# DrSleep/nas-segm-pytorch

Hardware: AMD Instinct MI355X
Metric: images/sec (fwd+bwd+optimizer step) WACV arch0 2048x1024 bs=4/GPU (higher is better)
Workload: dtype f32

## Files before the change

### include/nasseg.h

```cpp
#ifndef NASSEG_H
#define NASSEG_H

#include <stdint.h>

#ifdef __cplusplus
extern "C" {
#endif

const char* nasseg_last_error(void);
int nasseg_abi_version(void);
int nasseg_device_count(void);

int nasseg_dw_pack_weight(const float* w, float* wt, int C, int K, int flip, void* stream);
int nasseg_dwconv(const float* x, const float* wt, float* y, const float* in_scale,
                  const float* in_shift, int in_act, const float* scale, const float* shift, int act,
                  int B, int H, int W, int C, int Ho, int Wo, int K, int stride, int pad, int dil,
                  int transposed, float* stats, void* stream);
int nasseg_dwconv_strip_ok(int K, int stride, int dil);
int64_t nasseg_dwconv_stats_blocks(int B, int C, int Ho, int Wo, int K, int stride, int dil);
int nasseg_dwconv_bwd_data_bn(const float* dy, const float* wt, float* g, const float* z,
                              const float* scale, const float* shift, const float* mean,
                              const float* invstd, int act, int B, int H, int W, int C, int Ho,
                              int Wo, int K, int stride, int pad, int dil, int transposed,
                              float* stats, void* stream);
// ... 63 lines not shown
                            int dil, float* stats, void* stream);
int nasseg_conv_wgrad_lds3x3(int B, int Hs, int Ws, int K, int Ho, int Wo, int N, int kh, int kw, int stride,
                             int pad, int dil);
int64_t nasseg_conv_wgrad_workspace(int B, int Ho, int Wo, int N, int K, int kh, int kw);
int nasseg_wgrad_finalize_many(int count, const float* const* partial, float* const* dw,
                               const int* dims, void* stream);
int nasseg_conv_wgrad_many(int count, const int64_t* desc, void* stream);
int nasseg_dwconv_wgrad_many(int count, const int64_t* desc, void* stream);

int nasseg_conv_wgrad_bn(const float* x, int ldx, const float* g, int ldg, const float* z, int ldz, float* dz,
                         int lddz, float* dw, float* ws, const float* in_scale, const float* in_shift, int in_act,
                         const float* bn_scale, const float* bn_shift, const float* bn_mean, const float* bn_invstd,
                         const float* bn_sums, int bn_train, int bn_act, int B, int H, int W, int K, int N, void* stream);
int nasseg_conv_wgrad_bn_flat(const float* x, int ldx, const float* g, int ldg, const float* z, int ldz, float* dw,
                              float* ws, const float* bn_scale, const float* bn_shift, const float* bn_mean,
                              const float* bn_invstd, const float* bn_sums, int bn_train, int bn_act, int B, int Hs,
                              int Ws, int K, int Ho, int Wo, int N, int kh, int kw, int stride, int pad, int dil,
                              void* stream);
int nasseg_dwconv_wgrad_bn(const float* x, const float* g, const float* z, float* dz, float* dw, float* ws,
                           const float* in_scale, const float* in_shift, int in_act, const float* bn_scale, const float* bn_shift,
                           const float* bn_mean, const float* bn_invstd, const float* bn_sums, int bn_train, int bn_act,
                           int B, int H, int W, int C, int Ho, int Wo, int K, int stride, int pad, int dil,
                           void* stream);
int64_t nasseg_conv_pw_bwd_slabs(int B, int H, int W, int K, int N);
int64_t nasseg_conv_pw_bwd_reads_z(int B, int H, int W, int K, int N);
int64_t nasseg_conv_pw_bwd_kernel_id(int B, int H, int W, int K, int N, int z_null);
int64_t nasseg_conv_pw_bwd_rz_min_pixels(int64_t v);
int nasseg_conv_pw_bwd_bn(const float* x, const float* g, const float* z, const float* wb, float* dx, float* dw,
                          float* ws, const float* in_scale, const float* in_shift, int in_act, int dx_act,
                          const float* bn_scale, const float* bn_shift, const float* bn_mean, const float* bn_invstd,
                          const float* bn_sums, int bn_train, int bn_act, int B, int H, int W, int K, int N,
                          const float* in_mean, const float* in_invstd, float* dx_stats, const float* dx_res,
                          void* stream);
int nasseg_conv_wgrad(const float* x, int ldx, const float* dy, int lddy, float* dw, float* ws,
                      const float* in_scale, const float* in_shift, int in_act, int B, int Hs,
                      int Ws, int K, int Ho, int Wo, int N, int kh, int kw, int stride, int pad,
                      int dil, void* stream);

int64_t nasseg_colred_workspace(int S, int64_t R, int C);
int nasseg_colred(int mode, const float* a, int64_t lda, const float* b, int64_t ldb,
                  const float* c, int64_t ldc, float* out, float* ws, int S, int64_t R, int C,
                  float mul, void* stream);
int nasseg_bn_stats(const float* x, int64_t ldx, int64_t M, int C, float eps, float momentum,
                    const float* gamma, const float* beta, float* mean, float* invstd,
                    float* scale, float* shift, float* running_mean, float* running_var,
                    int64_t* num_batches_tracked, float* ws, void* stream);
int nasseg_bn_finalize(float* partial, int nblk, int64_t M, int C, float eps, float momentum,
                       const float* gamma, const float* beta, float* mean, float* invstd,
                       float* scale, float* shift, float* running_mean, float* running_var,
                       int64_t* num_batches_tracked, void* stream);
int nasseg_bn_eval_params(int C, float eps, const float* gamma, const float* beta,
                          const float* running_mean, const float* running_var, float* mean,
                          float* invstd, float* scale, float* shift, void* stream);
int nasseg_bn_bwd_reduce(const float* dy, int64_t lddy, const float* x, int64_t ldx, int64_t M,
                         int C, const float* scale, const float* shift, const float* mean,
                         const float* invstd, int act, float* sums, float* ws, void* stream);
int nasseg_rows_sum(float* partial, int nblk, int cols, float* out, void* stream);
int nasseg_bn_bwd_apply(const float* dy, const float* x, const float* scale, const float* shift,
                        const float* mean, const float* invstd, const float* sums, int64_t M,
                        int C, int train, int act, float* dx, void* stream);
int64_t nasseg_colred_rows(int S, int64_t R, int C);
int64_t nasseg_bn_bwd_apply_rows_max_bytes(void);
int nasseg_bn_bwd_reduce_rows(const float* dy, int64_t lddy, const float* x, int64_t ldx, int64_t M, int C,
                              const float* scale, const float* shift, const float* mean, const float* invstd, int act,
                              float* rows, void* stream);
int nasseg_bn_bwd_apply_rows(const float* dy, const float* x, const float* scale, const float* shift, const float* mean,
// ... 258 lines not shown
typedef struct nasseg_bf16_t {
  uint16_t v;
} nasseg_bf16_t;
int nasseg_to_bf16(const float* x, nasseg_bf16_t* y, int64_t n, void* stream);
int nasseg_from_bf16(const nasseg_bf16_t* x, float* y, int64_t n, void* stream);
int nasseg_bf16_irdw_stats(const nasseg_bf16_t* x, const float* w1, const float* in_scale, const float* in_shift,
                           int in_act, int B, int H, int W, int K, int C, float eps, float momentum, const float* gamma,
                           const float* beta, float* mean, float* invstd, float* scale, float* shift,
                           float* running_mean, float* running_var, int64_t* num_batches_tracked, float* ws,
                           void* stream);
int nasseg_bf16_irdw_fwd(const nasseg_bf16_t* x, const float* w1, const float* wdw, nasseg_bf16_t* z2,
                         const float* in_scale, const float* in_shift, int in_act, const float* bn1_scale,
                         const float* bn1_shift, int act1, int B, int H, int W, int K, int C, int Ho, int Wo, int stride,
                         float* stats, void* stream);
int nasseg_bf16_irdw_bwd(const nasseg_bf16_t* x, const float* w1, const nasseg_bf16_t* g, const nasseg_bf16_t* z2,
                         const float* wdw, int wdw_flipped, nasseg_bf16_t* ge, float* dw, float* ws,
                         const float* in_scale, const float* in_shift, int in_act, const float* bn1_scale,
                         const float* bn1_shift, const float* bn1_mean, const float* bn1_invstd, int act1,
                         const float* bn2_scale, const float* bn2_shift, const float* bn2_mean,
                         const float* bn2_invstd, const float* bn2_sums, int bn2_train, int bn2_act, int B, int H, int W,
                         int K, int C, int Ho, int Wo, int stride, float* stats, void* stream);
int nasseg_bf16_dwconv_bwd_bn(const nasseg_bf16_t* xz, const nasseg_bf16_t* g, const nasseg_bf16_t* z, const float* wt,
                              int wt_flipped, nasseg_bf16_t* ge, float* dw, float* ws, const float* in_scale, const float* in_shift,
                              const float* in_mean, const float* in_invstd, int in_act, const float* bn_scale,
                              const float* bn_shift, const float* bn_mean, const float* bn_invstd, const float* bn_sums,
                              int bn_train, int bn_act, int B, int H, int W, int C, int Ho, int Wo, int K, int stride,
                              int pad, int dil, float* stats, void* stream);
int nasseg_bf16_conv_pw_bwd_bn(const nasseg_bf16_t* x, const nasseg_bf16_t* g, const nasseg_bf16_t* z, const float* wb,
                               nasseg_bf16_t* dx, float* dw, float* ws, const float* in_scale, const float* in_shift,
                               int in_act, int dx_act, const float* bn_scale, const float* bn_shift, const float* bn_mean,
                               const float* bn_invstd, const float* bn_sums, int bn_train, int bn_act, int B, int H,
                               int W, int K, int N, const float* in_mean, const float* in_invstd, float* dx_stats,
                               const nasseg_bf16_t* dx_res, void* stream);
int nasseg_bf16_sepconv_fwd(const nasseg_bf16_t* x, const float* wdw, const float* wpw, nasseg_bf16_t* zdw,
                            nasseg_bf16_t* y, const float* in_scale, const float* in_shift, int in_act,
                            const float* out_scale, const float* out_shift, int out_act, int B, int H, int W, int C,
                            int Ho, int Wo, int N, int K, int stride, int pad, int dil, float* stats, void* stream);
int nasseg_bf16_affine_act(const nasseg_bf16_t* x, const float* scale, const float* shift, const nasseg_bf16_t* res,
                      nasseg_bf16_t* y, int64_t n, int C, int act, void* stream);
int nasseg_bf16_psum_bwd(const nasseg_bf16_t* dy, const nasseg_bf16_t* za, const float* tsa, int act_a, const float* ca,
                         nasseg_bf16_t* ga, float* part_a, const nasseg_bf16_t* zb, const float* tsb, int act_b,
                         const float* cb, nasseg_bf16_t* gb, float* part_b, float* cpart, int B, int H, int W, int C,
                         void* stream);
int nasseg_bf16_add_act2(const nasseg_bf16_t* xa, const float* sa, const float* ha, int act_a, const float* ca,
                         const nasseg_bf16_t* xb, const float* sb, const float* hb, int act_b, const float* cb,
                         nasseg_bf16_t* y, int64_t n, int C, void* stream);
int nasseg_bf16_bn_bwd_apply(const nasseg_bf16_t* dy, const nasseg_bf16_t* x, const float* scale, const float* shift,
                        const float* mean, const float* invstd, const float* sums, int64_t M,
                        int C, int train, int act, nasseg_bf16_t* dx, void* stream);
int nasseg_bf16_bn_bwd_reduce_rows(const nasseg_bf16_t* dy, int64_t lddy, const nasseg_bf16_t* x, int64_t ldx, int64_t M,
                                   int C, const float* scale, const float* shift, const float* mean, const float* invstd,
                                   int act, float* rows, void* stream);
int nasseg_bf16_bn_bwd_apply_rows(const nasseg_bf16_t* dy, const nasseg_bf16_t* x, const float* scale, const float* shift,
                                  const float* mean, const float* invstd, const float* rows, int nrows, float* sums_out,
                                  int64_t M, int C, int train, int act, nasseg_bf16_t* dx, void* stream);
int nasseg_bf16_grad_junction(const nasseg_bf16_t* g0, const nasseg_bf16_t* g1, const nasseg_bf16_t* g2,
                              const nasseg_bf16_t* g3, const nasseg_bf16_t* g4, const nasseg_bf16_t* g5,
                              const nasseg_bf16_t* g6, const nasseg_bf16_t* g7, int n, const nasseg_bf16_t* z,
                              const float* tstats, int act, nasseg_bf16_t* out, float* part, int B, int H, int W, int C,
                              void* stream);
int nasseg_bf16_axpby(const nasseg_bf16_t* a, const nasseg_bf16_t* b, const float* alpha, const float* beta, nasseg_bf16_t* y,
                 int64_t n, int C, int act, void* stream);
int nasseg_bf16_act_bwd(const nasseg_bf16_t* dy, const nasseg_bf16_t* ref, nasseg_bf16_t* dx, int64_t n, int act, void* stream);
int nasseg_bf16_fill(nasseg_bf16_t* y, int64_t n, float v, void* stream);
int nasseg_bf16_chan_copy(const nasseg_bf16_t* x, int64_t ldx, int xoff, nasseg_bf16_t* y, int64_t ldy, int yoff,
                     const nasseg_bf16_t* mref, int64_t ldm, int moff, int64_t P, int C, int act, int mact,
// ... 230 lines not shown
```

### nas-segm-pytorch_amd/csrc/conv_pwbwd.hip

```cpp
#include <atomic>
#include <cstdlib>
#include <type_traits>

#include "conv_common.h"

#if NASSEG_FP32_ONLY
std::atomic<int64_t> g_pw_rz_min_pixels{1 << 18};
#else
extern std::atomic<int64_t> g_pw_rz_min_pixels;
#endif

namespace {

#ifndef NASSEG_PW_CHUNK
#define NASSEG_PW_CHUNK 3
#endif
#ifndef NASSEG_PW_RECOMPUTE_Z
#define NASSEG_PW_RECOMPUTE_Z 1
#endif
constexpr int kPwTile = 64;
constexpr int kPwMaxTiles = 24;

struct PwArgs {
  const act_t* x;
  const act_t* g;
  const act_t* z;
  act_t* dx;
  float* partial;
  const float* wb;
  const float* in_scale;
  const float* in_shift;
  int in_act;
  const float* bn_scale;
  const float* bn_shift;
  const float* bn_mean;
  const float* bn_invstd;
  const float* bn_sums;
  int bn_train, bn_act;
  float invM;
  int dx_act;
  const float* in_mean;
  const float* in_invstd;
// ... 510 lines not shown
#pragma unroll
                for (int q = 0; q < NQ; ++q) acc[q] = mfma16(av, bv[q], acc[q]);
              }
            };
            switch (c) {
              case 0: dw_chunk(acc2[0]); break;
              case 1: dw_chunk(acc2[1]); break;
              case 2: if constexpr (KC > 2) dw_chunk(acc2[2]); break;
              case 3: if constexpr (KC > 3) dw_chunk(acc2[3]); break;
              case 4: if constexpr (KC > 4) dw_chunk(acc2[4]); break;
              default: if constexpr (KC > 5) dw_chunk(acc2[5]); break;
            }
          }
        };
        if (nq >= 4) mfma_phase(std::integral_constant<int, 4>());
        else if (nq == 3) mfma_phase(std::integral_constant<int, 3>());
        else if (nq == 2) mfma_phase(std::integral_constant<int, 2>());
        else mfma_phase(std::integral_constant<int, 1>());
      }
    }
  }
  if (own) {
    float* pout = a.partial + (int64_t)blockIdx.x * N * K;
#pragma unroll
    for (int c = 0; c < KC; ++c)
#pragma unroll
      for (int q = 0; q < 4; ++q)
#pragma unroll
        for (int r = 0; r < 4; ++r) {
          const int n = wave * 16 + 4 * kg + r, k = c * kPwChunk + q * 16 + j;
          if (n < N && k < K) pout[(int64_t)n * K + k] = acc2[c][q][r];
        }
  }
}

struct PwPlan {
  int ok, nt, kt, nslab, pix_per_slab, wide, rz;
};
inline int pw_round_nt(int nt) {
  const int allowed[] = {2, 3, 4, 6, 9, 12};
  for (int v : allowed)
    if (nt <= v) return v;
  return 0;
}
inline PwPlan pw_plan(int64_t M, int N, int K) {
  PwPlan p = {};
  if (N % 4 || K % 4 || N <= 0 || K <= 0 || M <= 0 || M >= 2147483647LL) return p;
  const int kt0 = cdiv(K, 16);
  p.kt = kt0 <= 1 ? 1 : (kt0 <= 2 ? 2 : (kt0 <= 4 ? 4 : 0));
  p.nt = pw_round_nt(cdiv(N, 16));
  if (!p.kt || !p.nt || p.nt * p.kt > kPwMaxTiles) {
    if (N > 64 || K > 384) return p;
    p.wide = 1;
    p.nt = cdiv(N, 16);
    p.kt = cdiv(K, kPwChunk);
  }
  const int64_t lds = p.wide ? (int64_t)(32 << 10)
                             : (int64_t)pw_lds_floats(p.nt, p.kt, pw_weight_in_lds(p.nt, p.kt)) * 4;
  int64_t s = lds > (40 << 10) ? 512 : 1024;
  const int64_t cap = (int64_t)((p.wide ? 64 : 16) << 20) / ((int64_t)N * K * 4);
  while (s > 1 && (s > cap || s > M / (4 * kPwTile))) s >>= 1;
  if (!p.wide && s < 256 && M / kPwTile > s) {
    s = M / kPwTile < 256 ? M / kPwTile : 256;
    if (s > cap) s = cap;
    if (s < 1) s = 1;
  }
// ... 128 lines not shown
    switch (id - kPwIdWide) {
      case 2: PW_WIDE(2); break;
      case 3: PW_WIDE(3); break;
      case 4: PW_WIDE(4); break;
      case 5: PW_WIDE(5); break;
      case 6: PW_WIDE(6); break;
      default: return nasseg_fail(NASSEG_ERR_UNSUPPORTED, "conv_pw_bwd_bn: no kernel with id %d", id);
    }
#undef PW_WIDE
    NASSEG_LAUNCH_CHECK("conv_pw_bwd_wide_kernel");
    if (!dw) return NASSEG_OK;
    const float* parts_w[1] = {ws};
    float* outs_w[1] = {dw};
    const int dims_w[5] = {p.nslab, 1, N, K, 0};
    return nasseg_wgrad_finalize_many(1, parts_w, outs_w, dims_w, stream);
  }
  switch (id) {
#define X(NT_, KT_) case pw_id(NT_, KT_, 1): pw_launch<NT_, KT_, true>(a, p.nslab, pro, s); break;
    PW_REBUILD(X)
#undef X
#define X(NT_, KT_) case pw_id(NT_, KT_, 0): pw_launch<NT_, KT_>(a, p.nslab, pro, s); break;
    PW_NARROW(X)
#undef X
    default: return nasseg_fail(NASSEG_ERR_UNSUPPORTED, "conv_pw_bwd_bn: no kernel with id %d", id);
  }
  NASSEG_LAUNCH_CHECK("conv_pw_bwd_kernel");
  if (!dw) return NASSEG_OK;
  const float* parts[1] = {ws};
  float* outs[1] = {dw};
  const int dims[5] = {p.nslab, 1, N, K, 0};
  return nasseg_wgrad_finalize_many(1, parts, outs, dims, stream);
}

}
```

### nas-segm-pytorch_amd/functional.py

```python
import collections
import ctypes
import os
import weakref

import numpy as np
import torch

from ._lib import LaunchProfiler, NassegError, current_stream, lib, ptr, require_device

ACT_NONE, ACT_RELU, ACT_RELU6 = 0, 1, 2
RED_SUM, RED_SUMSQ, RED_DOT2, RED_DOT1 = 0, 1, 3, 4


_BF16_PREFIX = "nasseg_bf16_"


def _k(name, t):
    if t.dtype == torch.float32:
        return name
    return _BF16_PREFIX + name[7:]


def _to_dtype(t, dtype):
    if t.dtype == dtype:
# ... 221 lines not shown

def _dense_wgrad(cur, dz, w, psc, psh, pact, geom):
    B, Hs, Ws, K, Ho, Wo, N, kh, kw, stride, pad, dil = geom
    dwt = torch.empty_like(w)
    ws = _ws(cur, lib.query("nasseg_conv_wgrad_workspace", B, Ho, Wo, N, K, kh, kw))
    flat = int(lib.query("nasseg_conv_fwd_pack_mode", K, kh, kw) == 2)
    if (deferred_wgrad.active and (B * Hs * Ws * K + B * Ho * Wo * N) * cur.element_size() <= _GROUP_WGRAD_BYTES
            and not (psc is None and psh is None and not pact
                     and lib.query("nasseg_conv_wgrad_lds3x3", B, Hs, Ws, K, Ho, Wo, N, kh, kw, stride, pad, dil))):
        desc = (ptr(cur), K, ptr(dz), N, ptr(ws), ptr(psc) or 0, ptr(psh) or 0, pact) + tuple(geom)
        _group_wgrad("nasseg_conv_wgrad_many", cur, (cur, dz, psc, psh, ws), desc,
                     _fin_entry(ws, dwt, kh * kw, N, K, flat))
        return dwt
    st = _wgrad_stream(cur, (cur, dz, psc, psh, ws))
    lib.call(_k("nasseg_conv_wgrad", cur), ptr(cur), K, ptr(dz), N, _finish_wgrad(ws, dwt, kh * kw, N, K, flat),
             ptr(ws), ptr(psc), ptr(psh), pact, *geom, st)
    return dwt


def _pw_bwd_slabs(kind, cur, z, w, stride, pad, need_dw, need_dx, i, ops):
    if not (FUSE_PW_BWD and kind == "dense" and need_dw and need_dx):
        return 0
    N, K, kh, kw = w.shape
    if not (kh == 1 and kw == 1 and stride == 1 and pad == 0):
        return 0
    if (cur.numel() + z.numel()) * cur.element_size() <= _PW_BWD_MIN_BYTES:
        return 0
    if K % 4 == 0 and i > 0 and ops[i - 1].has_bn and not (N >= K and K <= 64):
        return 0
    B, _, H, W = cur.shape
    if K > 64 and not (_PW_BWD_WIDE and B * H * W >= _PW_BWD_WIDE_MIN_PIXELS):
        return 0
    return lib.query("nasseg_conv_pw_bwd_slabs", B, H, W, K, N)


FUSE_DW_BWD = os.environ.get("NASSEG_FUSE_DW_BWD", "1") != "0"
_DW_BWD_MIN_BYTES = int(os.environ.get("NASSEG_DW_BWD_MIN_BYTES", 24 << 20))
_FLAT_WGRAD_BN_MIN_BYTES = 24 << 20


def _dw_bwd_rows(kind, cur, z, w, stride, pad, dil, need_dw, need_dx, i, ops):
    if not (FUSE_DW_BWD and kind == "dw" and need_dw and need_dx and i > 0 and ops[i - 1].has_bn):
        return 0
    if (cur.numel() + z.numel()) * cur.element_size() <= _DW_BWD_MIN_BYTES:
        return 0
    B, C, H, W = cur.shape
    return lib.query("nasseg_dwconv_bwd_bn_rows", B, C, H, W, w.shape[-1], stride, pad, dil)


def _flat_bn_ok(kind, need_dw, need_dx, psc, psh, pact, w, N, z):
    return (kind == "dense" and need_dw and not need_dx and psc is None and psh is None and not pact
            and w.shape[2] * w.shape[3] > 1 and N % 4 == 0
            and lib.query("nasseg_conv_fwd_pack_mode", w.shape[1], w.shape[2], w.shape[3]) == 2
            and z.numel() * z.element_size() > _FLAT_WGRAD_BN_MIN_BYTES)


def _wgrad_bn_ok(kind, cur, z, w, stride, pad, dil):
    if (cur.numel() + z.numel()) * cur.element_size() <= _GROUP_WGRAD_BYTES:
        return False
    K, N = cur.shape[1], z.shape[1]
    if kind == "dw":
        return K % 4 == 0 and bool(lib.query("nasseg_dwconv_strip_ok", w.shape[-1], stride, dil))
    return (w.shape[2] == 1 and w.shape[3] == 1 and stride == 1 and pad == 0 and K % 4 == 0 and N % 4 == 0)


def _wgrad_bn(kind, cur, g, z, w, psc, psh, pact, bn, geom):
# ... 336 lines not shown
        geom = (B, Ho, Wo, C, H, W, K, stride, pad, dil, 1)
    if bn is not None:
        nb = lib.query("nasseg_dwconv_bwd_data_bn_blocks", B, C, H, W, K, geom[7], geom[8], dil, geom[10])
        if nb > 0:
            z, scale, shift, mean, invstd, act = bn
            part = _rows_ws(dz, nb, C)
            lib.call(_k("nasseg_dwconv_bwd_data_bn", dz), ptr(dz), ptr(wt), ptr(dx), ptr(z), ptr(scale),
                     ptr(shift), ptr(mean), ptr(invstd), act, *geom, ptr(part), s)
            return dx, (part, nb)
    lib.call(_k("nasseg_dwconv", dz), ptr(dz), ptr(wt), ptr(dx), None, None, ACT_NONE, None, None,
             ACT_NONE, *geom, None, s)
    return dx, None


_IDENTITY = {}


def _identity_vectors(like, n):
    key = (like.device, (n + 1023) // 1024)
    ent = _IDENTITY.get(key)
    if ent is None:
        m = key[1] * 1024
        ent = (torch.ones(m, device=like.device, dtype=torch.float32),
               torch.zeros(m, device=like.device, dtype=torch.float32))
        _IDENTITY[key] = ent
    return ent


FUSE_RES_GRAD = os.environ.get("NASSEG_FUSE_RES_GRAD", "1") != "0"
FUSE_PW_BWD = os.environ.get("NASSEG_FUSE_PW_BWD", "1") != "0"
_PW_BWD_MIN_BYTES = int(os.environ.get("NASSEG_PW_BWD_MIN_BYTES", 24 << 20))
_PW_BWD_WIDE = os.environ.get("NASSEG_PW_BWD_WIDE", "1") == "1"
_PW_BWD_WIDE_MIN_PIXELS = 1 << 16
FUSE_BN_RELU_CONV = os.environ.get("NASSEG_FUSE_BN_RELU_CONV", "1") != "0"
FUSE_POOL_BN = os.environ.get("NASSEG_FUSE_POOL_BN", "1") != "0"
FUSE_CAT_REDUCE = os.environ.get("NASSEG_FUSE_CAT_REDUCE", "1") != "0"
FUSE_SEPCONV = os.environ.get("NASSEG_FUSE_SEPCONV", "1") != "0"
_PW_MIN_PIXELS = os.environ.get("NASSEG_PW_MIN_PIXELS")
_PWN_MODE = os.environ.get("NASSEG_PWN_MODE")


_SEPCONV_5X5_TRAIN_MAX = 10 << 20
_SEPCONV_5X5_TRAIN_MAX_WIDE = 4 << 20


def _sepconv_ok(x, w_dw, w_pw, op_dw, op_pw, needs_grad):
    B, C, H, W = x.shape
    k = w_dw.shape[-1]
    _, stride, pad, dil = op_dw[:4]
    N = w_pw.shape[0]
    if tuple(w_dw.shape) != (C, 1, k, k) or tuple(w_pw.shape) != (N, C, 1, 1):
        return False
    if op_pw[1:4] != (1, 0, 1):
        return False
    Ho, Wo = conv_out_size(H, k, stride, pad, dil), conv_out_size(W, k, stride, pad, dil)
    if Ho <= 0 or Wo <= 0:
        return False
    limit = _SEPCONV_5X5_TRAIN_MAX_WIDE if (C >= 64 and needs_grad) else _SEPCONV_5X5_TRAIN_MAX
    if k == 5 and B * Ho * Wo * C > limit and (needs_grad or C % 16 != 0):
        return False
    return lib.query("nasseg_sepconv_blocks", B, C, Ho, Wo, N, k, stride, dil) > 0


IRDW = os.environ.get("NASSEG_IRDW", "1") != "0"
_IRDW_MIN_PIXELS = int(os.environ.get("NASSEG_IRDW_MIN_PIXELS", 1 << 18))
_IRDW_S2_MAX_K = int(os.environ.get("NASSEG_IRDW_S2_MAX_K", 24))
# ... 162 lines not shown
        self.keep(i, OP_PLAIN, cur, pend, z, stats)
        if fold or not op.has_bn:
            return z, None, stats, (None if (fold and last) else res)
        if op.training:
            _bn_fill(parts, N, M, self.prm[i][1:], True, op.momentum, op.eps, z,
                     (part, nblk) if part is not None else None)
        return z, (scale, shift, op.act), stats, res

    def tail(self, cur, pend, stats, res):
        if self.cfg.pool is None:
            if pend is None:
                return (_axpby(cur, res, None, None) if res is not None else cur), None, None, False
            if self.cfg.defer and res is None and pend[0] is not None:
                return cur, stats, None, False
            return _affine_act(cur, pend[0], pend[1], res, pend[2]), None, None, False
        pk, ps, pp = self.cfg.pool
        B, N, Hc, Wc = cur.shape
        Hp, Wp = conv_out_size(Hc, pk, ps, pp, 1), conv_out_size(Wc, pk, ps, pp, 1)
        if Hp <= 0 or Wp <= 0:
            raise NassegError("max pooling output would be empty")
        psc, psh = (pend[0], pend[1]) if pend is not None else (None, None)
        if (res is not None or (pend is not None and pend[2] != ACT_NONE) or pk != 3 or pp != 1
                or ps not in (1, 2)):
            raise NassegError("conv_chain: the pooled tail serves conv + BatchNorm -> 3x3 max pooling only")
        y = _new(cur, B, N, Hp, Wp)
        pool_idx = torch.empty((B, Hp, Wp, N), device=cur.device, dtype=torch.uint8) if self.needs_grad else None
        lib.call(_k("nasseg_maxpool_bn_fwd", cur), ptr(cur), ptr(psc), ptr(psh), ptr(y), ptr(pool_idx), B, Hc,
                 Wc, N, Hp, Wp, ps, pp, self.s)
        return y, None, pool_idx, pend is not None


_Flow = collections.namedtuple("_Flow", "g rows masked dres in_masked")
_BnBwd = collections.namedtuple("_BnBwd", "scale shift mean invstd sums training act")
BWD_IRDW, BWD_DW_BN, BWD_FLAT_BN, BWD_PW_BN, BWD_WGRAD_BN, BWD_APPLY = range(6)


class _ChainBackward(collections.namedtuple("_ChainBackward", "ops recs meta need in_act0 fuse_res s")):

    def plan(self, i, need_dw, need_dx):
        op, r, (form, pact) = self.ops[i], self.recs[i], self.meta[i]
        if form == OP_IR_DW:
            return BWD_IRDW, 1
        if form == OP_IR_PW:
            B, K, H, W = r.x.shape
            return BWD_PW_BN, lib.query("nasseg_conv_pw_bwd_slabs", B, H, W, K, r.w.shape[0])
        nsl = _pw_bwd_slabs(op.kind, r.x, r.z, r.w, op.stride, op.pad, need_dw, need_dx, i, self.ops)
        if nsl > 0:
            return BWD_PW_BN, nsl
        rows = _dw_bwd_rows(op.kind, r.x, r.z, r.w, op.stride, op.pad, op.dil, need_dw, need_dx, i, self.ops)
        if rows > 0:
            return BWD_DW_BN, rows
        if _flat_bn_ok(op.kind, need_dw, need_dx, r.psc, r.psh, pact, r.w, r.w.shape[0], r.z):
            return BWD_FLAT_BN, 0
        if need_dw and _wgrad_bn_ok(op.kind, r.x, r.z, r.w, op.stride, op.pad, op.dil):
            return BWD_WGRAD_BN, 0
        return BWD_APPLY, 0

    def bn_head(self, i, fl, plan):
        op, r = self.ops[i], self.recs[i]
        N = r.w.shape[0]
        M = r.x.shape[0] * r.x.shape[2] * r.x.shape[3] if r.z is None else r.z.shape[0] * r.z.shape[2] * r.z.shape[3]
        mean, invstd, scale, shift = _bn_parts(r.stats, N)
        sums = _vec(fl.g, 2 * N)
        act_left = ACT_NONE if (fl.rows is not None or fl.masked) else op.act
        lazy_rows = fl.rows if (fl.rows is not None and plan == BWD_APPLY and _rows_small(fl.rows[1], N)) else None
        if fl.rows is not None and lazy_rows is None:
            lib.call("nasseg_rows_sum", ptr(fl.rows[0]), fl.rows[1], 2 * N, ptr(sums), self.s)
        elif fl.rows is None:
            lazy_rows = _bn_bwd_reduce(fl.g, r.z, scale, shift, mean, invstd, act_left, sums, M, N, plan == BWD_APPLY)
        dgamma = sums[N:2 * N] if self.need[3 + 6 * i + 1] else None
        dbeta = sums[0:N] if self.need[3 + 6 * i + 2] else None
        dz = None
        if plan == BWD_APPLY:
            dz = _bn_bwd_apply(fl.g, r.z, scale, shift, mean, invstd, sums, M, N, op.training, act_left,
                               torch.empty_like(r.z), lazy_rows)
        return _BnBwd(scale, shift, mean, invstd, sums, op.training, act_left), dz, dgamma, dbeta

    def producer_bn(self, i, K):
        if i > 0 and self.ops[i - 1].has_bn and K % 4 == 0:
            p = self.recs[i - 1]
            mean, invstd, scale, shift = _bn_parts(p.stats, K)
# ... 43 lines not shown
        op, r = self.ops[i], self.recs[i]
        Bc, K, H, W = r.x.shape
        N, _, kh, kw = r.w.shape
        _, _, Ho, Wo = r.z.shape
        dwt = torch.empty_like(r.w)
        ws = _ws(r.x, lib.query("nasseg_conv_wgrad_workspace", Bc, Ho, Wo, N, K, kh, kw))
        lib.call(_k("nasseg_conv_wgrad_bn_flat", r.x), ptr(r.x), K, ptr(fl.g), N, ptr(r.z), N,
                 _finish_wgrad(ws, dwt, kh * kw, N, K, 1), ptr(ws), ptr(bn.scale), ptr(bn.shift), ptr(bn.mean),
                 ptr(bn.invstd), ptr(bn.sums), int(bn.training), bn.act, Bc, H, W, K, Ho, Wo, N, kh, kw,
                 op.stride, op.pad, op.dil, self.s)
        return dwt, _Flow(None, None, False, fl.dres, fl.in_masked)

    def pw_bn(self, i, fl, bn, nsl):
        r, pact = self.recs[i], self.meta[i][1]
        Bc, K, H, W = r.x.shape
        N = r.w.shape[0]
        dwt = torch.empty_like(r.w)
        ws = _ws(r.x, nsl * N * K)
        g_in = _new(r.x, Bc, K, H, W)
        behind_bn = i > 0 and self.ops[i - 1].has_bn
        dx_act = pact if ((i == 0 and self.in_act0 and r.psc is None and r.psh is None) or behind_bn) else ACT_NONE
        part = pmu_ = pis_ = None
        skip_g = fl.dres if (self.fuse_res and i == 0 and K % 4 == 0) else None
        if behind_bn and K <= 64:
            pmu_, pis_ = _bn_parts(self.recs[i - 1].stats, K)[:2]
            part = _rows_ws(r.x, nsl, K)
        z_arg = r.z if (r.z is not None and lib.query("nasseg_conv_pw_bwd_reads_z", Bc, H, W, K, N)) else None
        lib.call(_k("nasseg_conv_pw_bwd_bn", r.x), ptr(r.x), ptr(fl.g), ptr(z_arg), ptr(r.wb), ptr(g_in),
                 _finish_wgrad(ws, dwt, 1, N, K, 0), ptr(ws), ptr(r.psc), ptr(r.psh), pact, dx_act,
                 ptr(bn.scale), ptr(bn.shift), ptr(bn.mean), ptr(bn.invstd), ptr(bn.sums), int(bn.training), bn.act,
                 Bc, H, W, K, N, ptr(pmu_), ptr(pis_), ptr(part), ptr(skip_g), self.s)
        return dwt, _Flow(g_in, (part, nsl) if part is not None else None, behind_bn,
                          fl.dres if skip_g is None else None, bool(dx_act) and i == 0)

    def generic(self, i, fl, bn, dz, need_dw, need_dx):
        op, r, pact = self.ops[i], self.recs[i], self.meta[i][1]
        Bc, K, H, W = r.x.shape
        _, N, Ho, Wo = r.z.shape
        kh, kw = r.w.shape[2], r.w.shape[3]
        bn_prev = self.producer_bn(i, K) if need_dx else None
        dw = op.kind == "dw"
        geom = ((Bc, H, W, K, Ho, Wo, kh, op.stride, op.pad, op.dil) if dw
                else (Bc, H, W, K, Ho, Wo, N, kh, kw, op.stride, op.pad, op.dil))
        dwt = None
        if bn is not None:
            dwt, dz = _wgrad_bn(op.kind, r.x, fl.g, r.z, r.w, r.psc, r.psh, pact, bn, geom if dw else (Bc, H, W, K, N))
        elif need_dw:
            dwt = (_dw_wgrad if dw else _dense_wgrad)(r.x, dz, r.w, r.psc, r.psh, pact, geom)
        if not need_dx:
            return dwt, _Flow(None, None, False, fl.dres, fl.in_masked)
        if dw:
            g, rows = _dw_backward_data(dz, r.wb, kh, (Bc, K, H, W), op.stride, op.pad, op.dil, bn_prev)
            return dwt, _Flow(g, rows, False, fl.dres, fl.in_masked)
        if bn_prev is not None:
            g = _new(r.x, Bc, K, H, W)
            zp, psc_, psh_, pmu_, pis_, pact_ = bn_prev
            pw1 = kh == 1 and kw == 1 and op.stride == 1 and op.pad == 0
            nb = lib.query("nasseg_conv_fwd_stats_blocks", Bc, H, W, K, N, 2 * int(pw1)) if pmu_ is not None else 0
            part = _rows_ws(r.x, nb, K) if nb else None
            lib.call(_k("nasseg_conv_bwd_data_bn", dz), ptr(dz), N, ptr(r.wb), ptr(g), K, ptr(zp), K,
                     ptr(psc_), ptr(psh_), ptr(pmu_), ptr(pis_), pact_, Bc, Ho, Wo, N, H, W,
                     K, kh, kw, op.stride, op.pad, op.dil, ptr(part), self.s)
            return dwt, _Flow(g, (part, nb), False, fl.dres, fl.in_masked)
        res = fl.dres if (self.fuse_res and i == 0) else None
        g = _dense_backward_data(dz, r.wb, _dense_dgrad_form(r.w, op.stride, op.pad, op.dil), (Bc, K, H, W), N, kh,
                                 kw, op.stride, op.pad, op.dil, res)
        return dwt, _Flow(g, None, False, fl.dres if res is None else None, fl.in_masked)

    def op(self, i, fl):
        need_dw, need_dx = self.need[3 + 6 * i], i > 0 or self.need[1]
        go_on = need_dw or need_dx
        bn, dz, dgamma, dbeta, plan, n = None, fl.g, None, None, BWD_APPLY, 0
        if self.ops[i].has_bn:
            plan, n = self.plan(i, need_dw, need_dx) if go_on else (None, 0)
            bn, dz, dgamma, dbeta = self.bn_head(i, fl, plan)
        if not go_on:
            return (None, dgamma, dbeta), fl._replace(g=None)
        if plan == BWD_IRDW:
            dwt, fl = self.irdw(i, fl, bn)
        elif plan == BWD_DW_BN:
            dwt, fl = self.dw_bn(i, fl, bn, n)
        elif plan == BWD_FLAT_BN:
            dwt, fl = self.flat_bn(i, fl, bn)
        elif plan == BWD_PW_BN:
            dwt, fl = self.pw_bn(i, fl, bn, n)
        else:
            dwt, fl = self.generic(i, fl, bn if plan == BWD_WGRAD_BN else None, dz, need_dw, need_dx)
        return (dwt, dgamma, dbeta), fl


class _ConvChain(torch.autograd.Function):

    @staticmethod
    def forward(ctx, cfg, x, residual, *tensors):
        res_is_x = residual is not None and residual is x
        x = _cl(x)
        ctx.set_materialize_grads(False)
        needs_grad = cfg.grad_mode and any(ctx.needs_input_grad)
        res = _cl(residual) if residual is not None else None
        pend = (None, None, cfg.in_act0) if cfg.in_act0 else None
        if cfg.in_pact is not None:
            pend = _scale_shift(tensors[-1], x.shape[1]) + (cfg.in_pact,)
        f = _ChainForward(cfg, x, tensors, needs_grad, ctx.needs_input_grad[1])
        ops, n = cfg.ops, len(cfg.ops)
        cur, stats, i = x, None, 0
        while i < n:
            if (needs_grad and i + 1 < n
                    and _irdw_ok(ops, i, f.w, cur, pend, i > 0 or ctx.needs_input_grad[1],
                                 ctx.needs_input_grad[3 + 6 * i] and ctx.needs_input_grad[3 + 6 * (i + 1)],
                                 ops[i].training)):
                cur, pend, stats = f.irdw(i, cur, pend)
                i += 2
            elif (ops[i].kind == "dw" and not ops[i].has_bn and i + 1 < n and FUSE_SEPCONV
                  and ops[i + 1].kind == "dense" and not (i + 2 == n and res is not None and not needs_grad)
                  and _sepconv_ok(cur, f.w[i], f.w[i + 1], ops[i], ops[i + 1], needs_grad)):
                cur, pend, stats, res = f.conv(i + 1, cur, pend, res, stage=i)
                i += 2
            else:
# ... 2043 lines not shown
                                   rows if g_lp is not None else None, g_lp, g_ent)
        grads = plan.split(flat)
        return (None, None, None) + tuple(g.view_as(p) if need else None
                                           for g, p, need in zip(grads, params, ctx.needs_input_grad[3:]))


def controller_rollout(plan, params, actions=None, rows=None):
    return _ControllerRollout.apply(plan, actions, rows, *params)


def controller_sample(plan, params, u):
    with torch.no_grad():
        entropy, _, _, sampled, sampled_lp = controller_forward(plan, [p.detach() for p in params], u=u)
    return sampled, sampled_lp, entropy


def controller_ppo_seed(log_prob, entropy, old_log_prob, adv, rows, clip_param, entropy_coef, acc, d_log_prob,
                        d_entropy):
    require_device(log_prob, entropy, old_log_prob, adv, rows, acc, d_log_prob, d_entropy)
    lib.call("nasseg_ctrl_ppo_seed", ptr(log_prob), ptr(entropy), ptr(old_log_prob), ptr(adv), ptr(rows),
             int(old_log_prob.numel()), int(log_prob.numel()), float(1.0 - clip_param), float(1.0 + clip_param),
             float(entropy_coef), ptr(acc), ptr(d_log_prob), ptr(d_entropy), current_stream())


def _apply_library_knobs():
    if _PW_MIN_PIXELS is not None:
        lib.query("nasseg_conv_pw_min_pixels", int(_PW_MIN_PIXELS))
        lib._memo.clear()
    if _PWN_MODE is not None:
        lib.query("nasseg_conv_pwn_mode", int(_PWN_MODE))
        lib._memo.clear()
    for env, fn in (("NASSEG_DW_WGRAD_LDS", "nasseg_dw_wgrad_lds"), ("NASSEG_CONV_DEEP_K", "nasseg_conv_deep_k"),
                    ("NASSEG_POOL_STRIP", "nasseg_pool_strip"),
                    ("NASSEG_PW_RZ_MIN_PIXELS", "nasseg_conv_pw_bwd_rz_min_pixels")):
        if os.environ.get(env) is not None:
            lib.query(fn, int(os.environ[env]))
            lib._memo.clear()


try:
    _apply_library_knobs()
except (OSError, NassegError):
    pass
```

Before: 306.4.

## Add fused contracting pointwise-conv backward kernel with BN, dgrad, wgrad and stats

Adds a new HIP kernel for 1x1 convolution backward where output channels are fewer than input channels (N<=32, 64<K<=192). In one pass over pixel slabs it applies the BatchNorm backward coefficients, computes the input gradient and the weight-gradient partials with MFMA, and accumulates the input-BN statistics, with register prefetch of the next tile. The Python backward planner routes eligible layers to this path by default above a pixel threshold, replacing the generic wgrad plus separate dgrad path. This costs extra LDS use and another kernel variant, and adds risk around the new planning conditions.

```diff
diff --git a/include/nasseg.h b/include/nasseg.h
--- a/include/nasseg.h
+++ b/include/nasseg.h
@@ -119,6 +119,15 @@
                           const float* bn_sums, int bn_train, int bn_act, int B, int H, int W, int K, int N,
                           const float* in_mean, const float* in_invstd, float* dx_stats, const float* dx_res,
                           void* stream);
+int64_t nasseg_conv_pw_bwd_contract_slabs(int B, int H, int W, int K, int N);
+int64_t nasseg_conv_pw_bwd_contract_kernel_id(int B, int H, int W, int K, int N);
+int64_t nasseg_conv_pw_bwd_contract_min_pixels(int64_t v);
+int nasseg_conv_pw_bwd_contract_bn(const float* x, const float* g, const float* z, const float* wb, float* dx,
+                                   float* dw, float* ws, const float* in_scale, const float* in_shift, int in_act,
+                                   int dx_act, const float* bn_scale, const float* bn_shift, const float* bn_mean,
+                                   const float* bn_invstd, const float* bn_sums, int bn_train, int bn_act, int B, int H,
+                                   int W, int K, int N, const float* in_mean, const float* in_invstd, float* dx_stats,
+                                   const float* dx_res, void* stream);
 int nasseg_conv_wgrad(const float* x, int ldx, const float* dy, int lddy, float* dw, float* ws,
                       const float* in_scale, const float* in_shift, int in_act, int B, int Hs,
                       int Ws, int K, int Ho, int Wo, int N, int kh, int kw, int stride, int pad,
@@ -443,6 +452,13 @@
                                const float* bn_invstd, const float* bn_sums, int bn_train, int bn_act, int B, int H,
                                int W, int K, int N, const float* in_mean, const float* in_invstd, float* dx_stats,
                                const nasseg_bf16_t* dx_res, void* stream);
+int nasseg_bf16_conv_pw_bwd_contract_bn(const nasseg_bf16_t* x, const nasseg_bf16_t* g, const nasseg_bf16_t* z,
+                                        const float* wb, nasseg_bf16_t* dx, float* dw, float* ws, const float* in_scale,
+                                        const float* in_shift, int in_act, int dx_act, const float* bn_scale,
+                                        const float* bn_shift, const float* bn_mean, const float* bn_invstd,
+                                        const float* bn_sums, int bn_train, int bn_act, int B, int H, int W, int K,
+                                        int N, const float* in_mean, const float* in_invstd, float* dx_stats,
+                                        const nasseg_bf16_t* dx_res, void* stream);
 int nasseg_bf16_sepconv_fwd(const nasseg_bf16_t* x, const float* wdw, const float* wpw, nasseg_bf16_t* zdw,
                             nasseg_bf16_t* y, const float* in_scale, const float* in_shift, int in_act,
                             const float* out_scale, const float* out_shift, int out_act, int B, int H, int W, int C,
diff --git a/nas-segm-pytorch_amd/csrc/conv_pwbwd.hip b/nas-segm-pytorch_amd/csrc/conv_pwbwd.hip
--- a/nas-segm-pytorch_amd/csrc/conv_pwbwd.hip
+++ b/nas-segm-pytorch_amd/csrc/conv_pwbwd.hip
@@ -8,6 +8,14 @@
 std::atomic<int64_t> g_pw_rz_min_pixels{1 << 18};
 #else
 extern std::atomic<int64_t> g_pw_rz_min_pixels;
+#endif
+#ifndef NASSEG_PW_CONTRACT_MIN_PIXELS
+#define NASSEG_PW_CONTRACT_MIN_PIXELS (1 << 17)
+#endif
+#if NASSEG_FP32_ONLY
+std::atomic<int64_t> g_pw_contract_min_pixels{NASSEG_PW_CONTRACT_MIN_PIXELS};
+#else
+extern std::atomic<int64_t> g_pw_contract_min_pixels;
 #endif
 
 namespace {
@@ -584,6 +592,229 @@
           if (n < N && k < K) pout[(int64_t)n * K + k] = acc2[c][q][r];
         }
   }
+}
+
+constexpr int kPcNT = 2;
+__host__ __device__ constexpr int pc_ktw(int KT) { return (KT + 3) / 4; }
+constexpr int kPcTile = 32;
+__host__ __device__ constexpr int pc_lds_floats(int KT) {
+  return kPcTile * (pw_lsn(kPcNT) + pw_lsk(KT)) + 4 * KT * 16 + 4 * kPcNT * 16;
+}
+template <int KT, bool PRO>
+__global__ __launch_bounds__(256, 2) void conv_pw_bwd_contract_kernel(PwArgs a) {
+  extern __shared__ float smem[];
+  constexpr int NT = kPcNT, KTW = pc_ktw(KT), LSN = pw_lsn(NT), LSK = pw_lsk(KT), KPc = KT * 16, KQ = KPc / 4;
+  constexpr int TP = kPcTile, SUBS = TP / 16, XU = (TP * KQ + 255) / 256;
+  float* dzt = smem;
+  float* zt = dzt + TP * LSN;
+  float* psc = zt + TP * LSK;
+  float* psh = psc + KPc;
+  float* pmu = psh + KPc;
+  float* pis = pmu + KPc;
+  float* cco = pis + KPc;
+  const int tid = threadIdx.x;
+  const int lane = tid & 63, wave = tid >> 6;
+  const int j = lane & 15, kg = lane >> 4;
+  const int N = a.N, K = a.K;
+  const int NS = a.NP >> 4;
+  for (int k = tid; k < KPc; k += 256) {
+    psc[k] = (PRO && a.in_scale && k < K) ? a.in_scale[k] : 1.f;
+    psh[k] = (PRO && a.in_shift && k < K) ? a.in_shift[k] : 0.f;
+    pmu[k] = (a.dx_stats && k < K) ? a.in_mean[k] : 0.f;
+    pis[k] = (a.dx_stats && k < K) ? a.in_invstd[k] : 0.f;
+  }
+  const ActSel pact = act_sel(a.in_act), bact = act_sel(a.bn_act), dact = act_sel(a.dx_act);
+  if (tid < NT * 16) {
+    float va = 0.f, vb = 0.f, vd = 0.f, vs = 0.f;
+    if (tid < N) {
+      const float sc = a.bn_scale[tid];
+      va = sc;
+      vs = a.bn_act ? a.bn_shift[tid] : 0.f;
+      if (a.bn_train) {
+        const float is = a.bn_invstd[tid], mu = a.bn_mean[tid];
+        const float s0 = a.bn_sums[tid] * a.invM, s1 = a.bn_sums[N + tid] * a.invM;
+        vb = -sc * is * s1;
+        vd = sc * fmaf(mu * is, s1, -s0);
+      }
+    }
+    cco[tid] = va;
+    cco[NT * 16 + tid] = vb;
+    cco[2 * NT * 16 + tid] = vd;
+    cco[3 * NT * 16 + tid] = vs;
+  }
+  const int gp = tid >> 3, gn = (tid & 7) * 4;
+  const bool gn_ok = gn < N;
+  bool own[KTW];
+  float4 wr[KTW][NT];
+  float pscj[KTW], pshj[KTW];
+#pragma unroll
+  for (int i = 0; i < KTW; ++i) {
+    const int kt = wave + 4 * i;
+    own[i] = kt < KT;
+    const int k = kt * 16 + j;
+    const bool kok = own[i] && k < K;
+#pragma unroll
+    for (int ns = 0; ns < NT; ++ns) {
+      const int n = ns * 16 + kg * 4;
+      wr[i][ns] = keep_if(ld4(a.wb + (int64_t)(kok ? k : 0) * N + (n < N ? n : 0)), kok && n < N);
+    }
+    pscj[i] = (PRO && a.in_scale && kok) ? a.in_scale[k] : 1.f;
+    pshj[i] = (PRO && a.in_shift && kok) ? a.in_shift[k] : 0.f;
+  }
+  f32x4 acc2[NT][KTW];
+  float4 sx[KTW], sq[KTW];
+#pragma unroll
+  for (int i = 0; i < KTW; ++i) {
+    sx[i] = sq[i] = f4zero();
+#pragma unroll
+    for (int nt = 0; nt < NT; ++nt) acc2[nt][i] = (f32x4){0.f, 0.f, 0.f, 0.f};
+  }
+  const int p_begin = blockIdx.x * a.pix_per_slab;
+  int p_end = p_begin + a.pix_per_slab;
+  if (p_end > a.M) p_end = a.M;
+
+  float4 gv, zv, xv[XU];
+  auto issue = [&](int t0) {
+    {
+      const int p = t0 + gp;
+      const int64_t off = (int64_t)(p < p_end ? p : p_end - 1) * N + (gn_ok ? gn : 0);
+      gv = lda4(a.g + off);
+      zv = lda4(a.z + off);
+    }
+#pragma unroll
+    for (int u = 0; u < XU; ++u) {
+      const int it = tid + 256 * u;
+      const int px = it / KQ, k = (it - px * KQ) * 4;
+      const int p = t0 + (px < TP ? px : TP - 1);
+      xv[u] = lda4(a.x + (int64_t)(p < p_end ? p : p_end - 1) * K + (k < K ? k : 0));
+    }
+  };
+  if (p_begin < p_end) issue(p_begin);
+  for (int t0 = p_begin; t0 < p_end; t0 += TP) {
+    __syncthreads();
+    {
+      const BnCoef kc = {ld4(cco + gn), ld4(cco + NT * 16 + gn), ld4(cco + 2 * NT * 16 + gn), ld4(cco + 3 * NT * 16 + gn)};
+      *reinterpret_cast<float4*>(&dzt[gp * LSN + gn]) =
+          keep_if(bn_coef_apply(gv, zv, kc, bact), t0 + gp < p_end && gn_ok);
+    }
+#pragma unroll
+    for (int u = 0; u < XU; ++u) {
+      const int it = tid + 256 * u;
+      const int px = it / KQ, k = (it - px * KQ) * 4;
+      if (px < TP) *reinterpret_cast<float4*>(&zt[px * LSK + k]) = keep_if(xv[u], t0 + px < p_end && k < K);
+    }
+    __syncthreads();
+    if (t0 + TP < p_end) issue(t0 + TP);
+#pragma unroll 4
+    for (int u = 0; u < TP / 4; ++u) {
+      const int pl = u * 4 + kg;
+      float av[NT], bv[KTW];
+#pragma unroll
+      for (int nt = 0; nt < NT; ++nt) av[nt] = dzt[pl * LSN + nt * 16 + j];
+#pragma unroll
+      for (int i = 0; i < KTW; ++i) {
+        if (!own[i]) continue;
+        const float v = zt[pl * LSK + (wave + 4 * i) * 16 + j];
+        bv[i] = PRO ? act_apply(fmaf(v, pscj[i], pshj[i]), pact) : v;
+      }
+#pragma unroll
+      for (int i = 0; i < KTW; ++i) {
+        if (!own[i]) continue;
+#pragma unroll
+        for (int nt = 0; nt < NT; ++nt) acc2[nt][i] = mfma16(av[nt], bv[i], acc2[nt][i]);
+      }
+    }
+#pragma unroll
+    for (int i = 0; i < KTW; ++i) {
+      if (!own[i]) continue;
+      const int k = (wave + 4 * i) * 16 + kg * 4;
+      const bool kok = k < K;
+      float4 rres[SUBS];
+      if (a.dx_res) {
+#pragma unroll
+        for (int sub = 0; sub < SUBS; ++sub) {
+          const int p = t0 + sub * 16 + j;
+          rres[sub] = lda4(a.dx_res + ((p < p_end && kok) ? (int64_t)p * K + k : 0));
+        }
+      }
+      f32x4 acc1[SUBS];
+#pragma unroll
+      for (int sub = 0; sub < SUBS; ++sub) acc1[sub] = (f32x4){0.f, 0.f, 0.f, 0.f};
+#pragma unroll
+      for (int ns = 0; ns < NT; ++ns) {
+        if (ns >= NS) continue;
+        float4 bv[SUBS];
+#pragma unroll
+        for (int sub = 0; sub < SUBS; ++sub)
+          bv[sub] = *reinterpret_cast<const float4*>(&dzt[(sub * 16 + j) * LSN + ns * 16 + kg * 4]);
+#pragma unroll
+        for (int sub = 0; sub < SUBS; ++sub) acc1[sub] = mfma16(wr[i][ns].x, bv[sub].x, acc1[sub]);
+#pragma unroll
+        for (int sub = 0; sub < SUBS; ++sub) acc1[sub] = mfma16(wr[i][ns].y, bv[sub].y, acc1[sub]);
+#pragma unroll
+        for (int sub = 0; sub < SUBS; ++sub) acc1[sub] = mfma16(wr[i][ns].z, bv[sub].z, acc1[sub]);
+#pragma unroll
+        for (int sub = 0; sub < SUBS; ++sub) acc1[sub] = mfma16(wr[i][ns].w, bv[sub].w, acc1[sub]);
+      }
+      const float4 sc4 = ld4(psc + k), sh4 = ld4(psh + k), mu4 = ld4(pmu + k), is4 = ld4(pis + k);
+#pragma unroll
+      for (int sub = 0; sub < SUBS; ++sub) {
+        const int pr = sub * 16 + j, p = t0 + pr;
+        const bool ok = p < p_end && kok;
+        const float4 zr = *reinterpret_cast<const float4*>(&zt[pr * LSK + k]);
+        float4 o = make_float4(acc1[sub][0], acc1[sub][1], acc1[sub][2], acc1[sub][3]);
+        if (a.dx_act) o = mask4(o, fma4(zr, sc4, sh4), dact);
+        if (ok) sta4(a.dx + (int64_t)p * K + k, a.dx_res ? add4(o, rres[sub]) : o);
+        const float4 gm = keep_if(as_stored4(o), ok);
+        sx[i] = add4(sx[i], gm);
+        sq[i] = fma4(gm, xhat4(zr, mu4, is4), sq[i]);
+      }
+    }
+  }
+  float* pout = a.partial + (int64_t)blockIdx.x * N * K;
+#pragma unroll
+  for (int i = 0; i < KTW; ++i) {
+    if (!own[i]) continue;
+    const int kt = wave + 4 * i;
+    if (a.dx_stats) {
+      const float vs[4] = {row16_allsum(sx[i].x), row16_allsum(sx[i].y), row16_allsum(sx[i].z), row16_allsum(sx[i].w)};
+      const float vq[4] = {row16_allsum(sq[i].x), row16_allsum(sq[i].y), row16_allsum(sq[i].z), row16_allsum(sq[i].w)};
+      float* po = a.dx_stats + (int64_t)blockIdx.x * 2 * K;
+#pragma unroll
+      for (int c = 0; c < 4; ++c) {
+        const int k = kt * 16 + kg * 4 + c;
+        if (j == 0 && k < K) {
+          po[k] = vs[c];
+          po[K + k] = vq[c];
+        }
+      }
+    }
+#pragma unroll
+    for (int nt = 0; nt < NT; ++nt)
+#pragma unroll
+      for (int r = 0; r < 4; ++r) {
+        const int n = nt * 16 + 4 * kg + r, k = kt * 16 + j;
+        if (n < N && k < K) pout[(int64_t)n * K + k] = acc2[nt][i][r];
+      }
+  }
+}
+
+struct PcPlan {
+  int ok, kt, nslab, pix_per_slab;
+};
+inline PcPlan pc_plan(int64_t M, int N, int K) {
+  PcPlan p = {};
+  if (N % 4 || K % 4 || N <= 0 || N > 16 * kPcNT || K <= 64 || K > 192 || M <= 0 || M >= 2147483647LL) return p;
+  const int kt0 = cdiv(K, 16);
+  p.kt = kt0 <= 6 ? 6 : (kt0 <= 9 ? 9 : 12);
+  int64_t s = 512;
+  while (s > 1 && s > M / (4 * kPwTile)) s >>= 1;
+  int64_t ppb = cdiv64(M, s);
+  ppb = (ppb + kPwTile - 1) / kPwTile * kPwTile;
+  p.pix_per_slab = (int)ppb;
+  p.nslab = (int)cdiv64(M, ppb);
+  p.ok = 1;
+  return p;
 }
 
 struct PwPlan {
@@ -778,4 +1009,73 @@
   return nasseg_wgrad_finalize_many(1, parts, outs, dims, stream);
 }
 
-}
+#if NASSEG_FP32_ONLY
+int64_t nasseg_conv_pw_bwd_contract_slabs(int B, int H, int W, int K, int N) {
+  if (B <= 0 || H <= 0 || W <= 0) return 0;
+  const int64_t M = (int64_t)B * H * W;
+  const PcPlan p = pc_plan(M, N, K);
+  return (p.ok && M >= g_pw_contract_min_pixels.load()) ? p.nslab : 0;
+}
+int64_t nasseg_conv_pw_bwd_contract_kernel_id(int B, int H, int W, int K, int N) {
+  if (B <= 0 || H <= 0 || W <= 0) return -1;
+  const PcPlan p = pc_plan((int64_t)B * H * W, N, K);
+  return p.ok ? p.kt : -1;
+}
+int64_t nasseg_conv_pw_bwd_contract_min_pixels(int64_t v) {
+  if (v < 0) return g_pw_contract_min_pixels.load();
+  return g_pw_contract_min_pixels.exchange(v);
+}
+#endif
+
+int NASSEG_FN(conv_pw_bwd_contract_bn)(const act_t* x, const act_t* g, const act_t* z, const float* wb, act_t* dx,
+                                       float* dw, float* ws, const float* in_scale, const float* in_shift,
+                                       int in_act, int dx_act, const float* bn_scale, const float* bn_shift,
+                                       const float* bn_mean, const float* bn_invstd, const float* bn_sums,
+                                       int bn_train, int bn_act, int B, int H, int W, int K, int N,
+                                       const float* in_mean, const float* in_invstd, float* dx_stats,
+                                       const act_t* dx_res, void* stream) {
+  NASSEG_REQUIRE(x && g && z && wb && dx && ws && bn_scale, "conv_pw_bwd_contract_bn: null tensor");
+  NASSEG_REQUIRE(!dx_stats || (in_mean && in_invstd), "conv_pw_bwd_contract_bn: dx_stats needs in_mean / in_invstd");
+  NASSEG_REQUIRE(!dx_res || !dx_stats, "conv_pw_bwd_contract_bn: dx_res needs no dx_stats");
+  NASSEG_REQUIRE((!bn_train || (bn_mean && bn_invstd && bn_sums)) && (!bn_act || bn_shift),
+                 "conv_pw_bwd_contract_bn: missing BatchNorm tensors");
+  NASSEG_REQUIRE(B > 0 && H > 0 && W > 0, "conv_pw_bwd_contract_bn: bad geometry");
+  NASSEG_REQUIRE(!dx_act || dx_act == in_act,
+                 "conv_pw_bwd_contract_bn: dx can only be masked with the derivative of the input activation");
+  const int64_t M = (int64_t)B * H * W;
+  const PcPlan p = pc_plan(M, N, K);
+  NASSEG_REQUIRE(p.ok, "conv_pw_bwd_contract_bn: no kernel for K=%d N=%d", K, N);
+  PwArgs a = {};
+  a.x = x; a.g = g; a.z = z; a.dx = dx; a.partial = ws; a.wb = wb;
+  a.in_scale = in_scale; a.in_shift = in_shift; a.in_act = in_act;
+  a.bn_scale = bn_scale; a.bn_shift = bn_shift; a.bn_mean = bn_mean; a.bn_invstd = bn_invstd;
+  a.bn_sums = bn_sums; a.bn_train = bn_train; a.bn_act = bn_act;
+  a.invM = (float)(1.0 / (double)M);
+  a.dx_act = dx_act;
+  a.in_mean = in_mean; a.in_invstd = in_invstd; a.dx_stats = dx_stats; a.dx_res = dx_res;
+  a.K = K; a.N = N; a.KP = (K + 15) & ~15; a.NP = (N + 15) & ~15;
+  a.M = (int)M; a.pix_per_slab = p.pix_per_slab;
+  const bool pro = in_scale || in_shift || in_act;
+  hipStream_t s = (hipStream_t)stream;
+#define PW_CONTRACT(KT_)                                                                                        \
+  do {                                                                                                          \
+    constexpr size_t lds = (size_t)pc_lds_floats(KT_) * sizeof(float);                                          \
+    static_assert(lds <= (64 << 10), "above the default limit of dynamic LDS");                                 \
+    if (pro) hipLaunchKernelGGL((conv_pw_bwd_contract_kernel<KT_, true>), dim3(p.nslab), dim3(256), lds, s, a);  \
+    else hipLaunchKernelGGL((conv_pw_bwd_contract_kernel<KT_, false>), dim3(p.nslab), dim3(256), lds, s, a);     \
+  } while (0)
+  switch (p.kt) {
+    case 6: PW_CONTRACT(6); break;
+    case 9: PW_CONTRACT(9); break;
+    default: PW_CONTRACT(12); break;
+  }
+#undef PW_CONTRACT
+  NASSEG_LAUNCH_CHECK("conv_pw_bwd_contract_kernel");
+  if (!dw) return NASSEG_OK;
+  const float* parts[1] = {ws};
+  float* outs[1] = {dw};
+  const int dims[5] = {p.nslab, 1, N, K, 0};
+  return nasseg_wgrad_finalize_many(1, parts, outs, dims, stream);
+}
+
+}
diff --git a/nas-segm-pytorch_amd/functional.py b/nas-segm-pytorch_amd/functional.py
--- a/nas-segm-pytorch_amd/functional.py
+++ b/nas-segm-pytorch_amd/functional.py
@@ -277,6 +277,16 @@
     if K > 64 and not (_PW_BWD_WIDE and B * H * W >= _PW_BWD_WIDE_MIN_PIXELS):
         return 0
     return lib.query("nasseg_conv_pw_bwd_slabs", B, H, W, K, N)
+
+
+def _pw_contract_slabs(kind, cur, w, stride, pad, need_dw, need_dx, i, ops):
+    if not (FUSE_PW_CONTRACT and kind == "dense" and need_dw and need_dx and i > 0 and ops[i - 1].has_bn):
+        return 0
+    N, K, kh, kw = w.shape
+    if not (kh == 1 and kw == 1 and stride == 1 and pad == 0 and N < K):
+        return 0
+    B, _, H, W = cur.shape
+    return lib.query("nasseg_conv_pw_bwd_contract_slabs", B, H, W, K, N)
 
 
 FUSE_DW_BWD = os.environ.get("NASSEG_FUSE_DW_BWD", "1") != "0"
@@ -679,6 +689,7 @@
 _PW_BWD_MIN_BYTES = int(os.environ.get("NASSEG_PW_BWD_MIN_BYTES", 24 << 20))
 _PW_BWD_WIDE = os.environ.get("NASSEG_PW_BWD_WIDE", "1") == "1"
 _PW_BWD_WIDE_MIN_PIXELS = 1 << 16
+FUSE_PW_CONTRACT = os.environ.get("NASSEG_FUSE_PW_CONTRACT", "1") != "0"
 FUSE_BN_RELU_CONV = os.environ.get("NASSEG_FUSE_BN_RELU_CONV", "1") != "0"
 FUSE_POOL_BN = os.environ.get("NASSEG_FUSE_POOL_BN", "1") != "0"
 FUSE_CAT_REDUCE = os.environ.get("NASSEG_FUSE_CAT_REDUCE", "1") != "0"
@@ -907,7 +918,7 @@
 
 _Flow = collections.namedtuple("_Flow", "g rows masked dres in_masked")
 _BnBwd = collections.namedtuple("_BnBwd", "scale shift mean invstd sums training act")
-BWD_IRDW, BWD_DW_BN, BWD_FLAT_BN, BWD_PW_BN, BWD_WGRAD_BN, BWD_APPLY = range(6)
+BWD_IRDW, BWD_DW_BN, BWD_FLAT_BN, BWD_PW_BN, BWD_PW_CONTRACT, BWD_WGRAD_BN, BWD_APPLY = range(7)
 
 
 class _ChainBackward(collections.namedtuple("_ChainBackward", "ops recs meta need in_act0 fuse_res s")):
@@ -922,6 +933,9 @@
         nsl = _pw_bwd_slabs(op.kind, r.x, r.z, r.w, op.stride, op.pad, need_dw, need_dx, i, self.ops)
         if nsl > 0:
             return BWD_PW_BN, nsl
+        nsl = _pw_contract_slabs(op.kind, r.x, r.w, op.stride, op.pad, need_dw, need_dx, i, self.ops)
+        if nsl > 0 and r.z is not None:
+            return BWD_PW_CONTRACT, nsl
         rows = _dw_bwd_rows(op.kind, r.x, r.z, r.w, op.stride, op.pad, op.dil, need_dw, need_dx, i, self.ops)
         if rows > 0:
             return BWD_DW_BN, rows
@@ -1031,6 +1045,21 @@
                  Bc, H, W, K, N, ptr(pmu_), ptr(pis_), ptr(part), ptr(skip_g), self.s)
         return dwt, _Flow(g_in, (part, nsl) if part is not None else None, behind_bn,
                           fl.dres if skip_g is None else None, bool(dx_act) and i == 0)
+
+    def pw_contract(self, i, fl, bn, nsl):
+        r, pact = self.recs[i], self.meta[i][1]
+        Bc, K, H, W = r.x.shape
+        N = r.w.shape[0]
+        dwt = torch.empty_like(r.w)
+        ws = _ws(r.x, nsl * N * K)
+        g_in = _new(r.x, Bc, K, H, W)
+        pmu_, pis_ = _bn_parts(self.recs[i - 1].stats, K)[:2]
+        part = _rows_ws(r.x, nsl, K)
+        lib.call(_k("nasseg_conv_pw_bwd_contract_bn", r.x), ptr(r.x), ptr(fl.g), ptr(r.z), ptr(r.wb), ptr(g_in),
+                 _finish_wgrad(ws, dwt, 1, N, K, 0), ptr(ws), ptr(r.psc), ptr(r.psh), pact, pact,
+                 ptr(bn.scale), ptr(bn.shift), ptr(bn.mean), ptr(bn.invstd), ptr(bn.sums), int(bn.training), bn.act,
+                 Bc, H, W, K, N, ptr(pmu_), ptr(pis_), ptr(part), None, self.s)
+        return dwt, _Flow(g_in, (part, nsl), True, fl.dres, fl.in_masked)
 
     def generic(self, i, fl, bn, dz, need_dw, need_dx):
         op, r, pact = self.ops[i], self.recs[i], self.meta[i][1]
@@ -1083,6 +1112,8 @@
             dwt, fl = self.flat_bn(i, fl, bn)
         elif plan == BWD_PW_BN:
             dwt, fl = self.pw_bn(i, fl, bn, n)
+        elif plan == BWD_PW_CONTRACT:
+            dwt, fl = self.pw_contract(i, fl, bn, n)
         else:
             dwt, fl = self.generic(i, fl, bn if plan == BWD_WGRAD_BN else None, dz, need_dw, need_dx)
         return (dwt, dgamma, dbeta), fl
@@ -3192,7 +3223,8 @@
         lib._memo.clear()
     for env, fn in (("NASSEG_DW_WGRAD_LDS", "nasseg_dw_wgrad_lds"), ("NASSEG_CONV_DEEP_K", "nasseg_conv_deep_k"),
                     ("NASSEG_POOL_STRIP", "nasseg_pool_strip"),
-                    ("NASSEG_PW_RZ_MIN_PIXELS", "nasseg_conv_pw_bwd_rz_min_pixels")):
+                    ("NASSEG_PW_RZ_MIN_PIXELS", "nasseg_conv_pw_bwd_rz_min_pixels"),
+                    ("NASSEG_PW_CONTRACT_MIN_PIXELS", "nasseg_conv_pw_bwd_contract_min_pixels")):
         if os.environ.get(env) is not None:
             lib.query(fn, int(os.environ[env]))
             lib._memo.clear()
```

Result: faster. 317.6 (median of 5 runs) (+3.6%).
